# fskovbo/OptimalControlMPS

Hardware: NVIDIA B200
Metric: cost+gradient evals/s (BH N=20 chi=100) (higher is better)
Workload: dtype complex128 (f64)

## Files before the change

optimalcontrolmps_b200/csrc/decomp.cu:

```cuda
#include <cstdio>
#include <cstdlib>
#include "ocmps_internal.h"

__device__ unsigned long long g_jac_dbg[8];
__device__ double g_jac_flops[2];

namespace {

constexpr int JAC_THREADS = 512;
constexpr int JAC_EPL = 8;
constexpr int JAC_NV_SMEM = 512;
constexpr int JAC_MAX_SWEEPS = 60;
constexpr int JAC_BLOCKED_ROWS = 64;
constexpr double JAC_TOL2 = 1e-28;
constexpr double DEFLATE_REL = 1e-30;
constexpr int NV_MAX = 2048;
constexpr int BJ_C = 8;
constexpr int BJ_TPP = 4;
constexpr int BJ_MAX_ROWS = 256;
constexpr int BJ_SLOTS = BJ_MAX_ROWS / 2;
constexpr int BJ_THREADS = BJ_SLOTS * BJ_TPP;
constexpr int BJ_MAX_EPL = 8;
constexpr int BJ_MIN_CAP = 112;

// ... 1344 lines not shown
        if (act && redo) { tnew = tail; if (hl == 0) sh.nref[hv] = tail; }
      }
      if (act && hl == 0) sh.ncur[hv] = tnew > 0.0 ? tnew : 0.0;
    }
    __syncthreads();
    QB_MARK(3)
  }
#ifdef OCMPS_JAC_TRACE
  if (tid == 0 && rank == 0 && nv >= 24)
    printf("JTQ kind %d blk %d nv %d len %d keff %d qr %lld : exchange %lld pull %lld norm+scalars %lld update %lld\n", a.kind, blk, nv, len, keff,
           (long long)(clock64() - t_qr0), tp[0], tp[1], tp[2], tp[3]);
#endif
  const int ldz = nv;
  for (int vl = warp; vl < nown; vl += BJ_THREADS / 32) {
    const int i = sh.posof[v0 + vl];
    const cplx* y = Yv + (size_t)vl * len;
    for (int c = lane; c < keff; c += 32) {
      cplx v = make_double2(0.0, 0.0);
      if (c < i) v = y[c];
      else if (c == i) v = make_double2(sh.rdr[c], sh.rdi[c]);
      Yb[(size_t)c * ldz + i] = v;
    }
  }
  if (rank == 0) {
    short* gperm = reinterpret_cast<short*>(b.scratch_d + 4 * NV_MAX) + B.p_off;
    for (int i = tid; i < nv; i += BJ_THREADS) gperm[i] = sh.pos2phys[i];
    if (tid == 0) {
      double* hF = b.scratch_d + 7 * NV_MAX;
      int* hK = reinterpret_cast<int*>(b.scratch_d + 7 * NV_MAX + OCMPS_MAX_BLK);
      hF[blk] = F;
      hK[blk] = -1;
      if (nv >= 64) { const long long t_now = clock64(); atomicAdd(&g_jac_dbg[5], (unsigned long long)(t_now - t_qr0)); atomicAdd(&g_jac_dbg[7], (unsigned long long)(t_now - t_qr0)); }
      hK[OCMPS_MAX_BLK + blk] = keff;
      hK[2 * OCMPS_MAX_BLK + blk] = ldz;
      const double nn = (double)len, mmv = (double)nv;
      atomicAdd(&g_jac_flops[0], 8.0 * nn * nn * mmv + (56.0 / 3.0) * nn * nn * nn);
      if (blk == 0) {
        const double dn = mode == 0 ? (double)w->n : (double)w->m, dm = mode == 0 ? (double)w->m : (double)w->n;
        atomicAdd(&g_jac_flops[1], 8.0 * dn * dn * dm + (56.0 / 3.0) * dn * dn * dn);
      }
    }
  }
  clus::cluster_sync();
}

struct BjShared {
  double2 xbuf[2][BJ_C][BJ_SLOTS];
  unsigned long long mbar[2];
  double nrm[BJ_MAX_ROWS];
  int rot, big;
};

__device__ __forceinline__ double2 bj_exchange(BjShared& sh, unsigned& xcount, unsigned rank, int nslots, int slot, int lane, double x, double y) {
  const unsigned b = xcount & 1u, par = (xcount >> 1) & 1u;
  ++xcount;
  const unsigned mb = clus::smem_u32(&sh.mbar[b]);
  if (lane == 0 && slot < nslots) {
    sh.xbuf[b][rank][slot] = make_double2(x, y);
    const unsigned la = clus::smem_u32(&sh.xbuf[b][rank][slot]);
#pragma unroll
    for (unsigned p = 1; p < (unsigned)BJ_C; ++p) {
      const unsigned peer = (rank + p) % BJ_C;
      clus::st_async_v2(clus::mapa(la, peer), x, y, clus::mapa(mb, peer));
    }
  }
  clus::mbar_wait(mb, par);
  if (threadIdx.x == 0) clus::mbar_expect(mb, (unsigned)((BJ_C - 1) * nslots * 16));
  __syncwarp();
  double sx = 0.0, sy = 0.0;
  if (slot < nslots) {
#pragma unroll
    for (int r = 0; r < BJ_C; ++r) { const double2 v = sh.xbuf[b][r][slot]; sx += v.x; sy += v.y; }
  }
  return make_double2(sx, sy);
}

template <int TPP, int EPL>
__device__ void bj_run(DecompBuffers& b, const DecompBlock& B, int keff, int ldz, double F, cplx* __restrict__ Rs, BjShared& sh) {
  const int tid = threadIdx.x, slot = tid / TPP, lane = tid % TPP;
  const unsigned rank = clus::cluster_rank();
  const int nv = B.nv;
  const int w = (nv + BJ_C - 1) / BJ_C;
  const int c0 = (int)rank * w;
  constexpr int WP = (TPP * EPL) % 8 == 0 ? TPP * EPL + 4 : ((TPP * EPL) % 8 == 4 ? TPP * EPL : TPP * EPL + (12 - (TPP * EPL) % 8) % 8);
  const cplx* Yb = b.ywork + b.ywork_half + B.ws_off;
  cplx* Ya = b.ywork + B.ws_off;
  const short* perm = reinterpret_cast<const short*>(b.scratch_d + 4 * NV_MAX) + B.p_off;
  const double thr = F * DEFLATE_REL;
  unsigned xcount = 0;
  for (int e = tid; e < keff * WP; e += BJ_THREADS) {
    const int r = e / WP, cl = e % WP, c = c0 + cl;
    Rs[e] = (cl < w && c < nv) ? Yb[(size_t)r * ldz + c] : make_double2(0.0, 0.0);
  }
  __syncthreads();
  const int npad = (keff + 1) & ~1, nslots = npad >> 1, mm = npad - 1;
  cplx ra[EPL], rb[EPL];
  auto load_row = [&](cplx (&r)[EPL], int row) {
    const cplx* z = Rs + (row >= 0 ? row : 0) * WP + lane;
#pragma unroll
    for (int e = 0; e < EPL; ++e) r[e] = row >= 0 ? z[TPP * e] : make_double2(0.0, 0.0);
  };
  auto store_row = [&](const cplx (&r)[EPL], int row) {
    if (row < 0) return;
    cplx* z = Rs + row * WP + lane;
#pragma unroll
    for (int e = 0; e < EPL; ++e) z[TPP * e] = r[e];
  };
  auto lanes_sum = [&](double v) {
#pragma unroll
    for (int o = TPP / 2; o > 0; o >>= 1) v += __shfl_xor_sync(0xffffffffu, v, o);
    return v;
  };
  auto exact_norms = [&]() {
    const int x = 2 * slot < keff ? 2 * slot : -1, y = 2 * slot + 1 < keff ? 2 * slot + 1 : -1;
    load_row(ra, x);
    load_row(rb, y);
    double sa = 0.0, sb = 0.0;
#pragma unroll
    for (int e = 0; e < EPL; ++e) { sa += ra[e].x * ra[e].x + ra[e].y * ra[e].y; sb += rb[e].x * rb[e].x + rb[e].y * rb[e].y; }
    sa = lanes_sum(sa); sb = lanes_sum(sb);
    const double2 t = bj_exchange(sh, xcount, rank, nslots, slot, lane, sa, sb);
    if (lane == 0) { if (x >= 0) sh.nrm[x] = t.x; if (y >= 0) sh.nrm[y] = t.y; }
  };
  bool converged = keff < 2;
#ifdef OCMPS_JAC_TRACE
  long long tq[3] = {0, 0, 0};
  long long tql = clock64();
  int nrounds = 0;
#define BJ_MARK(i) { const long long tn = clock64(); tq[i] += tn - tql; tql = tn; }
#else
#define BJ_MARK(i)
#endif
  for (int sweep = 0; sweep < JAC_MAX_SWEEPS && !converged; ++sweep) {
    exact_norms();
    if (tid == 0) { sh.rot = 0; sh.big = 0; }
    __syncthreads();
    for (int R = 0; R < npad - 1; ++R) {
      int p = -1, q = -1;
      if (slot < nslots) {
        p = R + slot; if (p >= mm) p -= mm;
        q = R - slot; if (q < 0) q += mm;
        if (slot == 0) q = npad - 1;
        if (p > q) { const int t = p; p = q; q = t; }
        if (q >= keff) { p = -1; q = -1; }
      }
      const bool act = p >= 0;
      load_row(ra, p);
      load_row(rb, q);
      const double aa = act ? sh.nrm[p] : 0.0, bb = act ? sh.nrm[q] : 0.0;
      double c0r = 0.0, c0i = 0.0, c1r = 0.0, c1i = 0.0;
#pragma unroll
      for (int e = 0; e < EPL; ++e) {
        const double pr = ra[e].x * rb[e].x + ra[e].y * rb[e].y;
        const double pi = ra[e].x * rb[e].y - ra[e].y * rb[e].x;
        if (e & 1) { c1r += pr; c1i += pi; } else { c0r += pr; c0i += pi; }
      }
      const double pre = lanes_sum(c0r + c1r), pim = lanes_sum(c0i + c1i);
      BJ_MARK(0)
      const double2 cc = bj_exchange(sh, xcount, rank, nslots, slot, lane, pre, pim);
      BJ_MARK(1)
      if (act) {
        const double cre = cc.x, cim = cc.y;
        const double c2 = cre * cre + cim * cim;
        if (aa <= thr || bb <= thr) {
          if (aa <= thr && aa > 0.0) {
#pragma unroll
            for (int e = 0; e < EPL; ++e) ra[e] = make_double2(0.0, 0.0);
            store_row(ra, p);
            if (lane == 0) sh.nrm[p] = 0.0;
          }
          if (bb <= thr && bb > 0.0) {
#pragma unroll
            for (int e = 0; e < EPL; ++e) rb[e] = make_double2(0.0, 0.0);
            store_row(rb, q);
            if (lane == 0) sh.nrm[q] = 0.0;
          }
        } else if (c2 > JAC_TOL2 * aa * bb) {
          const double dd = 0.5 * (bb - aa);
          const double xh = dd * dd + c2;
          const double ih = rsqrt(xh);
          const double h = xh * ih;
          const double sdh = fabs(dd) + h;
          const double wv = rsqrt(2.0 * h * sdh);
          const double cs = sdh * wv;
          const double sgw = dd >= 0.0 ? wv : -wv;
          const double sr = sgw * cre, si = sgw * cim;
#pragma unroll
          for (int e = 0; e < EPL; ++e) {
            const cplx u = ra[e], v = rb[e];
            ra[e] = make_double2(cs * u.x - (sr * v.x + si * v.y), cs * u.y - (sr * v.y - si * v.x));
            rb[e] = make_double2(cs * v.x + (sr * u.x - si * u.y), cs * v.y + (sr * u.y + si * u.x));
          }
          store_row(ra, p);
          store_row(rb, q);
          if (lane == 0) {
            const double trr = c2 * (sgw * wv) * (2.0 * h);
            const double a1 = aa - trr, b1 = bb + trr;
            sh.nrm[p] = a1 > 0.0 ? a1 : 0.0;
            sh.nrm[q] = b1 > 0.0 ? b1 : 0.0;
            sh.rot = 1;
            if (c2 > 1e-16 * aa * bb) sh.big = 1;
          }
        }
      }
      __syncthreads();
      BJ_MARK(2)
#ifdef OCMPS_JAC_TRACE
      ++nrounds;
#endif
    }
    converged = (sh.rot == 0) || (sh.big == 0);
    __syncthreads();
    if (!converged && sweep == JAC_MAX_SWEEPS - 1 && tid == 0 && rank == 0) atomicOr(b.status, OCMPS_ST_NOCONV);
    if (tid == 0 && rank == 0) { atomicAdd(&g_jac_dbg[0], 1ull); atomicMax(&g_jac_dbg[2], (unsigned long long)(sweep + 1)); if (nv >= 64) atomicAdd(&g_jac_dbg[3], 1ull); if (nv >= 64 && sweep == 0) atomicAdd(&g_jac_dbg[4], 1ull); }
  }
#ifdef OCMPS_JAC_TRACE
  if (tid == 0 && rank == 0 && nv >= 24 && nrounds > 0)
    printf("JTB nv %d keff %d EPL %d rounds %d per round: load+dot %lld exchange %lld rotate+sync %lld\n", nv, keff, EPL, nrounds, tq[0] / nrounds, tq[1] / nrounds,
           tq[2] / nrounds);
#endif
  exact_norms();
  __syncthreads();
  for (int v = slot; v < nv; v += BJ_THREADS / TPP) {
    if (v < keff) {
      const double sq = sh.nrm[v];
      const double inv = sq > 0.0 ? rsqrt(sq) : 0.0;
      for (int cl = lane; cl < w; cl += TPP) {
        const int c = c0 + cl;
        if (c < nv) { const cplx u = Rs[v * WP + cl]; Ya[(size_t)v * nv + (int)perm[c]] = make_double2(u.x * inv, u.y * inv); }
      }
      if (lane == 0 && rank == 0) b.P[B.p_off + v] = sq;
    } else if (lane == 0 && rank == 0) {
      b.P[B.p_off + v] = 0.0;
    }
  }
}

__global__ void __launch_bounds__(BJ_THREADS) jacobi_big_kernel(DecompArgs a, DecompBuffers b) {
  extern __shared__ __align__(16) unsigned char smem_raw[];
  __shared__ BjShared sh;
  const DecompWork* w = b.dw;
  const int blk = blockIdx.x / BJ_C;
  if (blk >= w->nblocks) return;
  if (w->blk[blk].nv > BJ_MAX_ROWS || w->blk[blk].len > BJ_MAX_ROWS) return;
  const int* hK = reinterpret_cast<const int*>(b.scratch_d + 7 * NV_MAX + OCMPS_MAX_BLK);
  const int keff = hK[OCMPS_MAX_BLK + blk];
  if (keff < 0) return;
  const int ldz = hK[2 * OCMPS_MAX_BLK + blk];
  const DecompBlock B = w->blk[blk];
  const double F = (b.scratch_d + 7 * NV_MAX)[blk];
  const int tid = threadIdx.x;
  const int nslots = ((keff + 1) & ~1) >> 1;
  if (tid == 0) {
    clus::mbar_init(clus::smem_u32(&sh.mbar[0]), 1);
    clus::mbar_init(clus::smem_u32(&sh.mbar[1]), 1);
    asm volatile("fence.mbarrier_init.release.cluster;" ::: "memory");
    clus::mbar_expect(clus::smem_u32(&sh.mbar[0]), (unsigned)((BJ_C - 1) * nslots * 16));
    clus::mbar_expect(clus::smem_u32(&sh.mbar[1]), (unsigned)((BJ_C - 1) * nslots * 16));
  }
  __syncthreads();
  clus::cluster_sync();
  const long long t0 = clock64();
  cplx* Rs = reinterpret_cast<cplx*>(smem_raw);
  const int wcols = (B.nv + BJ_C - 1) / BJ_C;
  if (keff <= BJ_THREADS / 8 * 2) {
    switch ((wcols + 7) / 8) {
      case 1: bj_run<8, 1>(b, B, keff, ldz, F, Rs, sh); break;
      case 2: bj_run<8, 2>(b, B, keff, ldz, F, Rs, sh); break;
      case 3: bj_run<8, 3>(b, B, keff, ldz, F, Rs, sh); break;
      default: bj_run<8, 4>(b, B, keff, ldz, F, Rs, sh); break;
    }
  } else {
    switch ((wcols + 3) / 4) {
      case 1: bj_run<4, 1>(b, B, keff, ldz, F, Rs, sh); break;
      case 2: bj_run<4, 2>(b, B, keff, ldz, F, Rs, sh); break;
      case 3: bj_run<4, 3>(b, B, keff, ldz, F, Rs, sh); break;
      case 4: bj_run<4, 4>(b, B, keff, ldz, F, Rs, sh); break;
      case 5: bj_run<4, 5>(b, B, keff, ldz, F, Rs, sh); break;
      case 6: bj_run<4, 6>(b, B, keff, ldz, F, Rs, sh); break;
      case 7: bj_run<4, 7>(b, B, keff, ldz, F, Rs, sh); break;
      default: bj_run<4, 8>(b, B, keff, ldz, F, Rs, sh); break;
    }
  }
  clus::cluster_sync();
  if (tid == 0 && clus::cluster_rank() == 0) {
    atomicAdd(&g_jac_dbg[1], 1ull);
    const long long t1 = clock64();
    if (B.nv >= 64) { atomicAdd(&g_jac_dbg[6], (unsigned long long)(t1 - t0)); atomicAdd(&g_jac_dbg[7], (unsigned long long)(t1 - t0)); }
#ifdef OCMPS_JAC_TRACE
    if (B.nv >= 24) printf("JT3 kind %d blk %d nv %d keff %d jac %lld\n", a.kind, blk, B.nv, keff, (long long)(t1 - t0));
#endif
  }
}

constexpr int RC_C = 4;
constexpr int RC_NBLK = 2 * RC_C;
constexpr int RC_ROWS = JAC_BLOCKED_ROWS / RC_NBLK;
constexpr int RC_WORK_THREADS = 16 * RC_ROWS;
constexpr int RC_MIN_ROWS = 40;

__device__ unsigned long long g_rc_dbg[2];

struct RcShared {
  double nrm[2][2][RC_ROWS];
  int flags[2][RC_C];
  int rot, big;
};

__device__ __forceinline__ void rc_blocks(int R, int s, int& P, int& Q) {
  constexpr int mm = RC_NBLK - 1;
  int p = R + s; if (p >= mm) p -= mm;
  int q = R - s; if (q < 0) q += mm;
  if (s == 0) q = RC_NBLK - 1;
  P = p; Q = q;
}

__device__ __forceinline__ void rc_bar() { asm volatile("bar.sync 1, %0;" ::"n"(RC_WORK_THREADS) : "memory"); }

template <int EPL>
__device__ __forceinline__ void rc_block_round(cplx* __restrict__ Z0, cplx* __restrict__ Z1, double* n0, double* n1, int rb, int base0, int base1,
                                               int keff, double thr, bool intra, int* s_rot, int* s_big) {
  constexpr int ldz = 16 * EPL;
  const int tid = threadIdx.x, hl = tid & 15, h = tid >> 4;
  cplx ra[EPL], rb_[EPL];
  double na = 0.0, nb = 0.0;
  auto load_row = [&](cplx (&r)[EPL], double& n, const cplx* Z, const double* nz, int row) {
    const cplx* z = Z + (row >= 0 ? row : 0) * ldz + hl;
#pragma unroll
    for (int e = 0; e < EPL; ++e) r[e] = row >= 0 ? z[16 * e] : make_double2(0.0, 0.0);
    n = row >= 0 ? nz[row] : 0.0;
  };
  auto store_row = [&](const cplx (&r)[EPL], double n, cplx* Z, double* nz, int row) {
    cplx* z = Z + row * ldz + hl;
#pragma unroll
    for (int e = 0; e < EPL; ++e) z[16 * e] = r[e];
    if (hl == 0) nz[row] = n;
  };
  if (intra) {
    const int X = h / (RC_ROWS / 2), j = h % (RC_ROWS / 2);
    cplx* Z = X ? Z1 : Z0;
    double* nz = X ? n1 : n0;
    const int base = X ? base1 : base0;
    const int rbp = (rb + 1) & ~1, m = rbp - 1;
    for (int r = 0; r < m; ++r) {
      int p = r + j; if (p >= m) p -= m;
      int q = r - j; if (q < 0) q += m;
      if (j == 0) q = m;
      const bool act = 2 * j < rbp && p < rb && q < rb && base + p < keff && base + q < keff;
      load_row(ra, na, Z, nz, act ? p : -1);
      load_row(rb_, nb, Z, nz, act ? q : -1);
      jac_rotate<EPL>(ra, rb_, na, nb, act, thr, hl, s_rot, s_big);
      if (act) { store_row(ra, na, Z, nz, p); store_row(rb_, nb, Z, nz, q); }
      rc_bar();
    }
  }
  const bool has_a = h < rb && base0 + h < keff;
  load_row(ra, na, Z0, n0, has_a ? h : -1);
  for (int t = 0; t < rb; ++t) {
    int jb = h + t; if (jb >= rb) jb -= rb;
    const bool act = has_a && base1 + jb < keff;
    load_row(rb_, nb, Z1, n1, act ? jb : -1);
    jac_rotate<EPL>(ra, rb_, na, nb, act, thr, hl, s_rot, s_big);
    if (act) store_row(rb_, nb, Z1, n1, jb);
    rc_bar();
  }
  if (has_a) store_row(ra, na, Z0, n0, h);
}

template <int EPL>
__device__ __forceinline__ void rc_run(const DecompArgs& a, const DecompBuffers& b, int blk, int keff, unsigned rank, cplx* __restrict__ Zs, RcShared& sh) {
  constexpr int ldz = 16 * EPL;
  constexpr int BLK = RC_ROWS * ldz;
  const int tid = threadIdx.x, lane = tid & 31, warp = tid >> 5, nwarps = JAC_THREADS / 32;
  const DecompBlock B = b.dw->blk[blk];
  const int nv = B.nv;
  const int rb = (keff + RC_NBLK - 1) / RC_NBLK;
  const double F = (b.scratch_d + 7 * NV_MAX)[blk];
  const double thr = F * DEFLATE_REL;
  const cplx* Yb = b.ywork + b.ywork_half + B.ws_off;
  auto zb = [&](int buf, int k) { return Zs + (2 * buf + k) * BLK; };
  const long long t_jac0 = clock64();
  int P, Q;
  rc_blocks(0, (int)rank, P, Q);
  for (int e = tid; e < 2 * BLK; e += JAC_THREADS) {
    const int k = e / BLK, r = (e % BLK) / ldz, c = e % ldz;
    const int row = (k ? Q : P) * rb + r;
    Zs[e] = (r < rb && row < keff) ? Yb[row * ldz + c] : make_double2(0.0, 0.0);
  }
  __syncthreads();
  int cur = 0;
  bool done = false;
#ifdef OCMPS_JAC_TRACE
  long long t_work = 0, t_xchg = 0;
  int nrounds = 0, nxchg = 0;
#endif
  for (int sweep = 0; sweep < JAC_MAX_SWEEPS && !done; ++sweep) {
    for (int lr = warp; lr < 2 * RC_ROWS; lr += nwarps) {
      const int k = lr / RC_ROWS, r = lr % RC_ROWS;
      const cplx* y = zb(cur, k) + r * ldz;
      double s = 0.0;
      for (int c = lane; c < nv; c += 32) { const cplx u = y[c]; s += u.x * u.x + u.y * u.y; }
      s = warp_sum(s);
      if (lane == 0) sh.nrm[cur][k][r] = s;
    }
    if (tid == 0) { sh.rot = 0; sh.big = 0; }
    __syncthreads();
    for (int R = 0; R < RC_NBLK - 1; ++R) {
#ifdef OCMPS_JAC_TRACE
      const long long tw0 = clock64();
#endif
      if (tid < RC_WORK_THREADS) rc_block_round<EPL>(zb(cur, 0), zb(cur, 1), sh.nrm[cur][0], sh.nrm[cur][1], rb, P * rb, Q * rb, keff, thr, R == 0, &sh.rot, &sh.big);
      __syncthreads();
#ifdef OCMPS_JAC_TRACE
      const long long tw1 = clock64();
      t_work += tw1 - tw0;
      nrounds += rb + (R == 0 ? ((rb + 1) & ~1) - 1 : 0);
#endif
      const bool last = R == RC_NBLK - 2;
      if (last && tid < RC_C) {
        const int f = (sh.rot ? 1 : 0) | (sh.big ? 2 : 0);
        asm volatile("st.shared::cluster.u32 [%0], %1;" ::"r"(clus::mapa(clus::smem_u32(&sh.flags[sweep & 1][rank]), (unsigned)tid)), "r"(f) : "memory");
      }
      clus::cluster_sync();
      if (last) {
        int any = 0;
#pragma unroll
        for (int r = 0; r < RC_C; ++r) any |= sh.flags[sweep & 1][r];
        done = !(any & 1) || !(any & 2);
        if (tid == 0 && rank == 0) {
          atomicAdd(&g_jac_dbg[0], 1ull); atomicMax(&g_jac_dbg[2], (unsigned long long)(sweep + 1)); atomicAdd(&g_rc_dbg[1], 1ull);
          if (nv >= 64) atomicAdd(&g_jac_dbg[3], 1ull);
          if (nv >= 64 && sweep == 0) atomicAdd(&g_jac_dbg[4], 1ull);
          if (!done && sweep == JAC_MAX_SWEEPS - 1) atomicOr(b.status, OCMPS_ST_NOCONV);
        }
        if (done || sweep == JAC_MAX_SWEEPS - 1) break;
      }
      int NP, NQ;
      rc_blocks(last ? 0 : R + 1, (int)rank, NP, NQ);
      unsigned src0 = 0, src1 = 0, nsrc0 = 0, nsrc1 = 0;
      for (int s = 0; s < RC_C; ++s) {
        int p, q;
        rc_blocks(R, s, p, q);
        const unsigned zp = clus::mapa(clus::smem_u32(zb(cur, 0)), (unsigned)s), zq = clus::mapa(clus::smem_u32(zb(cur, 1)), (unsigned)s);
        const unsigned np = clus::mapa(clus::smem_u32(sh.nrm[cur][0]), (unsigned)s), nq = clus::mapa(clus::smem_u32(sh.nrm[cur][1]), (unsigned)s);
        if (p == NP) { src0 = zp; nsrc0 = np; }
        if (q == NP) { src0 = zq; nsrc0 = nq; }
        if (p == NQ) { src1 = zp; nsrc1 = np; }
        if (q == NQ) { src1 = zq; nsrc1 = nq; }
      }
      for (int e = tid; e < 2 * rb * ldz; e += JAC_THREADS) {
        const int k = e >= rb * ldz, o = e - k * rb * ldz;
        double xr, xi;
        asm volatile("ld.shared::cluster.v2.f64 {%0, %1}, [%2];" : "=d"(xr), "=d"(xi) : "r"((k ? src1 : src0) + (unsigned)o * 16u) : "memory");
        zb(cur ^ 1, k)[o] = make_double2(xr, xi);
      }
      if (tid < 2 * RC_ROWS) {
        const int k = tid / RC_ROWS, r = tid % RC_ROWS;
        double x;
        asm volatile("ld.shared::cluster.f64 %0, [%1];" : "=d"(x) : "r"((k ? nsrc1 : nsrc0) + (unsigned)r * 8u) : "memory");
        sh.nrm[cur ^ 1][k][r] = x;
      }
      __syncthreads();
#ifdef OCMPS_JAC_TRACE
      t_xchg += clock64() - tw1;
      ++nxchg;
#endif
      cur ^= 1; P = NP; Q = NQ;
    }
  }
  const long long t_jac1 = clock64();
  const short* perm = reinterpret_cast<const short*>(b.scratch_d + 4 * NV_MAX) + B.p_off;
  cplx* Ya = b.ywork + B.ws_off;
  for (int lr = warp; lr < 2 * RC_ROWS; lr += nwarps) {
    const int k = lr / RC_ROWS, r = lr % RC_ROWS, v = (k ? Q : P) * rb + r;
    if (r >= rb || v >= keff) continue;
    const cplx* y = zb(cur, k) + r * ldz;
    double s = 0.0;
    for (int c = lane; c < nv; c += 32) { const cplx u = y[c]; s += u.x * u.x + u.y * u.y; }
    s = warp_sum(s);
    const double inv = s > 0.0 ? rsqrt(s) : 0.0;
    for (int c = lane; c < nv; c += 32) {
      const cplx u = y[c];
      Ya[v * nv + (int)perm[c]] = make_double2(u.x * inv, u.y * inv);
    }
    if (lane == 0) b.P[B.p_off + v] = s;
  }
  if (rank == 0) for (int v = keff + tid; v < nv; v += JAC_THREADS) b.P[B.p_off + v] = 0.0;
  if (tid == 0 && rank == 0) {
    atomicAdd(&g_jac_dbg[1], 1ull);
    atomicAdd(&g_rc_dbg[0], 1ull);
    if (nv >= 64) {
      atomicAdd(&g_jac_dbg[6], (unsigned long long)(t_jac1 - t_jac0));
      atomicAdd(&g_jac_dbg[7], (unsigned long long)(t_jac1 - t_jac0));
    }
#ifdef OCMPS_JAC_TRACE
    if (nv >= 24)
      printf("JTR kind %d blk %d nv %d keff %d rb %d jac %lld : rotation rounds %d, %lld clk per round; block exchanges %d, %lld clk each\n", a.kind, blk, nv,
             keff, rb, t_jac1 - t_jac0, nrounds, nrounds ? t_work / nrounds : 0ll, nxchg, nxchg ? t_xchg / nxchg : 0ll);
#endif
  }
}

__global__ void __launch_bounds__(JAC_THREADS) jacobi_rows_cluster_kernel(DecompArgs a, DecompBuffers b, int smem_elems) {
  extern __shared__ __align__(16) unsigned char smem_raw[];
  __shared__ RcShared sh;
  const int blk = (int)blockIdx.x / RC_C;
  const unsigned rank = clus::cluster_rank();
  const int keff = rot_handover_rows(b, blk, smem_elems);
  if (keff < 0) return;
  if (keff < RC_MIN_ROWS) {
    if (rank == 0) jacobi_rot_block(a, b, blk, keff, smem_raw);
    return;
  }
  cplx* Zs = reinterpret_cast<cplx*>(smem_raw);
  switch ((b.dw->blk[blk].nv + 15) >> 4) {
    case 1: rc_run<1>(a, b, blk, keff, rank, Zs, sh); break;
    case 2: rc_run<2>(a, b, blk, keff, rank, Zs, sh); break;
    case 3: rc_run<3>(a, b, blk, keff, rank, Zs, sh); break;
    case 4: rc_run<4>(a, b, blk, keff, rank, Zs, sh); break;
    case 5: rc_run<5>(a, b, blk, keff, rank, Zs, sh); break;
    case 6: rc_run<6>(a, b, blk, keff, rank, Zs, sh); break;
    case 7: rc_run<7>(a, b, blk, keff, rank, Zs, sh); break;
    default: rc_run<8>(a, b, blk, keff, rank, Zs, sh); break;
  }
}

__global__ void __launch_bounds__(1024) truncate_kernel(DecompArgs a, DecompBuffers b, TruncParams tp) {
  __shared__ double cP[NV_MAX];
  __shared__ double sSorted[NV_MAX];
  __shared__ short cQ[NV_MAX], cI[NV_MAX], cI2[NV_MAX];
  __shared__ unsigned char sKeep[NV_MAX];
  __shared__ int sBlkOff[OCMPS_MAX_BLK + 1];
  __shared__ double sWarp[32];
  __shared__ int sWarpCnt[33];
  __shared__ double s_docut, s_kept;
  __shared__ int s_nfinal;
  DecompWork* w = b.dw;
  const int nv = w->nvtot;
  const int nblocks = w->nblocks;
  const int tid = threadIdx.x, lane = tid & 31, warp = tid >> 5;
  for (int i = tid; i < nblocks; i += blockDim.x) sBlkOff[i] = w->blk[i].p_off;
  if (tid == 0) { s_nfinal = 0; s_docut = 0.0; }
  const int i0 = 2 * tid, i1 = i0 + 1;
  const double p0 = i0 < nv ? b.P[i0] : 0.0, p1 = i1 < nv ? b.P[i1] : 0.0;
  const int f0 = p0 > 0.0, f1 = p1 > 0.0;
  int incl = f0 + f1;
#pragma unroll
  for (int o = 1; o < 32; o <<= 1) { const int up = __shfl_up_sync(0xffffffffu, incl, o); if (lane >= o) incl += up; }
  if (lane == 31) sWarpCnt[warp + 1] = incl;
  if (tid == 0) sWarpCnt[0] = 0;
  __syncthreads();
  if (warp == 0) {
    int v = sWarpCnt[lane + 1];
#pragma unroll
    for (int o = 1; o < 32; o <<= 1) { const int up = __shfl_up_sync(0xffffffffu, v, o); if (lane >= o) v += up; }
    sWarpCnt[lane + 1] = v;
  }
  __syncthreads();
  const int nnz = sWarpCnt[32];
  {
    int k = sWarpCnt[warp] + incl - f0 - f1;
    if (f0) { cP[k] = p0; cQ[k] = (short)b.vecq[i0]; cI[k] = (short)i0; ++k; }
    if (f1) { cP[k] = p1; cQ[k] = (short)b.vecq[i1]; cI[k] = (short)i1; }
  }
  __syncthreads();
  {
    int tpe = 1;
    while (tpe < 8 && nnz * tpe * 2 <= (int)blockDim.x) tpe *= 2;
    const int sub = tid & (tpe - 1);
    for (int k0 = 0; k0 < nnz; k0 += (int)blockDim.x / tpe) {
      const int k = k0 + tid / tpe;
      const bool in = k < nnz;
      const double pk = in ? cP[k] : 0.0;
      int rank = 0;
      if (in)
        for (int j = sub; j < nnz; j += tpe) {
          const double pj = cP[j];
          rank += (pj > pk) || (pj == pk && j < k);
        }
      for (int o = 1; o < tpe; o <<= 1) rank += __shfl_xor_sync(0xffffffffu, rank, o);
      if (in && sub == 0) sSorted[rank] = pk;
    }
  }
  __syncthreads();
  const int origm = nv;
  const int e0 = nnz - 1 - 2 * tid, e1 = e0 - 1;
  const double v0 = e0 >= 0 ? sSorted[e0] : 0.0, v1 = e1 >= 0 ? sSorted[e1] : 0.0;
  {
    double run = v0 + v1;
#pragma unroll
    for (int o = 1; o < 32; o <<= 1) { const double up = __shfl_up_sync(0xffffffffu, run, o); if (lane >= o) run += up; }
    if (lane == 31) sWarp[warp] = run;
    __syncthreads();
    if (warp == 0) {
      double ws = sWarp[lane];
#pragma unroll
      for (int o = 1; o < 32; o <<= 1) { const double up = __shfl_up_sync(0xffffffffu, ws, o); if (lane >= o) ws += up; }
      sWarp[lane] = ws;
    }
    __syncthreads();
    const double base = warp > 0 ? sWarp[warp - 1] : 0.0;
    const double inc = base + run;
    if (e0 >= 0) sSorted[e0] = inc - v1;
    if (e1 >= 0) sSorted[e1] = inc;
  }
  __syncthreads();
  {
    const double total_w = nnz > 0 ? sSorted[0] : 0.0;
    const double scale = tp.rel_cutoff ? (total_w == 0.0 ? 1.0 : total_w) : 1.0;
    const double cut = tp.cutoff * scale;
    const int nmax = (tp.maxm < origm ? tp.maxm : origm) - 1;
    int best = 0;
    if (cut <= 0.0) {
      best = nmax > 0 ? nmax : 0;
    } else {
      const int lim = nmax < nnz - 1 ? nmax : nnz - 1;
      for (int n = tid; n <= lim; n += blockDim.x)
        if (n < tp.minm || sSorted[n] >= cut) best = n > best ? n : best;
      if (tp.minm - 1 > best && tp.minm - 1 <= nmax) best = tp.minm - 1;
    }
    if (best > 0) atomicMax(&s_nfinal, best);
  }
  __syncthreads();
  {
    const int m = s_nfinal + 1;
    if (tid == 0) { sWarp[0] = 0.0; sWarp[1] = 0.0; }
    __syncthreads();
    if (e0 == m) sWarp[0] = v0;
    if (e1 == m) sWarp[0] = v1;
    if (e0 == m - 1) sWarp[1] = v0;
    if (e1 == m - 1) sWarp[1] = v1;
    __syncthreads();
    if (tid == 0) {
      double docut = 0.0;
      if (origm == 1) {
        docut = sWarp[1] / 2.0;
      } else if (origm > 1 && m < origm) {
        const double pm = sWarp[0], pm1 = sWarp[1];
        docut = (pm + pm1) / 2.0;
        if (fabs(pm - pm1) < 1e-3 * pm1) docut += 1e-3 * pm1;
      }
      s_docut = docut;
    }
    __syncthreads();
  }
  const double docut = s_docut;
  {
    const int ka = 2 * tid, kb = ka + 1;
    const int fa = ka < nnz && cP[ka] > docut, fb = kb < nnz && cP[kb] > docut;
    if (ka < nnz) sKeep[ka] = (unsigned char)fa;
    if (kb < nnz) sKeep[kb] = (unsigned char)fb;
    int inc = fa + fb;
#pragma unroll
    for (int o = 1; o < 32; o <<= 1) { const int up = __shfl_up_sync(0xffffffffu, inc, o); if (lane >= o) inc += up; }
    __syncthreads();
    if (lane == 31) sWarpCnt[warp + 1] = inc;
    if (tid == 0) sWarpCnt[0] = 0;
    __syncthreads();
    if (warp == 0) {
      int v = sWarpCnt[lane + 1];
#pragma unroll
      for (int o = 1; o < 32; o <<= 1) { const int up = __shfl_up_sync(0xffffffffu, v, o); if (lane >= o) v += up; }
      sWarpCnt[lane + 1] = v;
    }
    __syncthreads();
    const int base = sWarpCnt[warp] + inc - fa - fb;
    if (ka < nnz) cI2[ka] = (short)base;
    if (kb < nnz) cI2[kb] = (short)(base + fa);
  }
  __syncthreads();
  const int total = sWarpCnt[32];
  int* inv_blk = b.pos + NV_MAX;
  int* inv_v = b.pos + 2 * NV_MAX;
  double part = 0.0;
  for (int k = tid; k < nnz; k += blockDim.x) {
    if (!sKeep[k]) continue;
    const int qk = cQ[k];
    const double pk = cP[k];
    int rank = 0, j = k - 1;
    for (; j >= 0 && cQ[j] == qk; --j) rank += sKeep[j] && cP[j] >= pk;
    const int pos0 = cI2[j + 1];
    for (j = k + 1; j < nnz && cQ[j] == qk; ++j) rank += sKeep[j] && cP[j] > pk;
    const int pos = pos0 + rank;
    if (pos < tp.cap) {
      const int i = cI[k];
      a.qNew[pos] = qk;
      int bi = 0;
      while (bi + 1 < nblocks && sBlkOff[bi + 1] <= i) ++bi;
      inv_blk[pos] = bi;
      inv_v[pos] = i - sBlkOff[bi];
      part += pk;
    }
  }
  {
#pragma unroll
    for (int o = 16; o > 0; o >>= 1) part += __shfl_xor_sync(0xffffffffu, part, o);
    __syncthreads();
    if (lane == 0) sWarp[warp] = part;
    __syncthreads();
    if (tid == 0) {
      double t = 0.0;
      for (int i = 0; i < 32; ++i) t += sWarp[i];
      s_kept = t;
    }
    __syncthreads();
  }
  if (tid == 0) {
    int k = total;
    if (k == 0 && nv > 0) {
      k = 1;
      a.qNew[0] = b.vecq[0];
      inv_blk[0] = 0;
      inv_v[0] = 0;
    }
    if (k > tp.cap) { atomicOr(b.status, OCMPS_ST_CAPACITY); k = tp.cap; }
    w->newdim = k;
    *a.dimNew = k;
    const double kept = s_kept;
    double scale = 1.0;
    if (tp.normalize) {
      const double nrm = sqrt(kept);
      if (nrm > 1e-16) scale = 1.0 / nrm;
    }
    w->scale = scale;
    const int n = w->n, m = w->m;
    GemmDesc g1;
    g1.pad = 0;
    g1.A = g1.B = nullptr; g1.C = nullptr; g1.M = g1.N = g1.K = 0; g1.lda = g1.ldb = g1.ldc = 1; g1.opA = g1.opB = 0;
    if (a.kind == DK_ORTH_LEFT) {
      const int far = a.D * (*a.dimNb);
      g1.A = a.partner; g1.opA = 0; g1.lda = m;
      g1.B = a.nb_in; g1.opB = 0; g1.ldb = far;
      g1.C = a.nb_out; g1.ldc = far; g1.M = k; g1.N = far; g1.K = m;
    } else if (a.kind == DK_ORTH_RIGHT) {
      const int far = a.D * (*a.dimNb);
      g1.A = a.nb_in; g1.opA = 0; g1.lda = n;
      g1.B = a.partner; g1.opB = 0; g1.ldb = k;
      g1.C = a.nb_out; g1.ldc = k; g1.M = far; g1.N = k; g1.K = n;
    }
    b.descs[1] = g1;
  }
}

constexpr int BUILD_THREADS = 512;
__global__ void __launch_bounds__(BUILD_THREADS) build_factors_kernel(DecompArgs a, DecompBuffers b) {
  extern __shared__ __align__(16) unsigned char bsm[];
  __shared__ double red[BUILD_THREADS / 32];
  __shared__ double s_inv;
  const DecompWork* w = b.dw;
  const int k = w->newdim;
  const int kk = blockIdx.x;
  if (kk >= k) return;
  const int n = w->n, m = w->m, ld = w->ld, mode = w->mode;
  const int* comp_blk = b.comp_idx + NV_MAX;
  const int* comp_rank = b.comp_idx + 2 * NV_MAX;
  const int* vec_blk = b.vec_idx + NV_MAX;
  const int* vec_rank = b.vec_idx + 2 * NV_MAX;
  const int bi = b.pos[NV_MAX + kk], j = b.pos[2 * NV_MAX + kk];
  const DecompBlock B = w->blk[bi];
  const int nv = B.nv, len = B.len;
  const cplx* Zj = b.ywork + B.ws_off + (size_t)j * nv;
  const double sigma = sqrt(b.P[B.p_off + j]) * w->scale;
  cplx* zs = reinterpret_cast<cplx*>(bsm);
  cplx* out = zs + nv;
  int* vidx = reinterpret_cast<int*>(out + len);
  int* cidx = vidx + nv;
  const int tid = threadIdx.x, lane = tid & 31, wp = tid >> 5;
  constexpr int NW = BUILD_THREADS / 32;
  for (int v = tid; v < nv; v += BUILD_THREADS) { zs[v] = Zj[v]; vidx[v] = b.vec_idx[B.vec_off + v]; }
  for (int c = tid; c < len; c += BUILD_THREADS) cidx[c] = b.comp_idx[B.comp_off + c];
// ... 328 lines not shown
```

Baseline: 0.9277.

## Replace per-round cluster barrier with push-based st.async exchange and mbarrier handshakes

Measured after the change: 0.9425, median of 6. 1.6% higher.

```diff
diff --git a/optimalcontrolmps_b200/csrc/decomp.cu b/optimalcontrolmps_b200/csrc/decomp.cu
--- a/optimalcontrolmps_b200/csrc/decomp.cu
+++ b/optimalcontrolmps_b200/csrc/decomp.cu
@@ -1670,7 +1670,9 @@
 __device__ unsigned long long g_rc_dbg[2];
 
 struct RcShared {
+  unsigned long long full[2];
   double nrm[2][2][RC_ROWS];
+  unsigned freed[RC_C];
   int flags[2][RC_C];
   int rot, big;
 };
@@ -1681,6 +1683,27 @@
   int q = R - s; if (q < 0) q += mm;
   if (s == 0) q = RC_NBLK - 1;
   P = p; Q = q;
+}
+
+__device__ __forceinline__ void rc_holder(int R, int X, int& s, int& k) {
+  s = 0; k = 0;
+  for (int r = 0; r < RC_C; ++r) {
+    int p, q;
+    rc_blocks(R, r, p, q);
+    if (p == X) { s = r; k = 0; }
+    if (q == X) { s = r; k = 1; }
+  }
+}
+
+template <int EPL>
+__device__ __forceinline__ unsigned rc_in_bytes(int Rn, int rank, int rb) {
+  const int Rp = Rn == 0 ? RC_NBLK - 2 : Rn - 1;
+  int P, Q, s, k;
+  rc_blocks(Rn, rank, P, Q);
+  unsigned n = 0;
+  rc_holder(Rp, P, s, k); if (s != rank) ++n;
+  rc_holder(Rp, Q, s, k); if (s != rank) ++n;
+  return n * (unsigned)(rb * 16 * EPL * 16 + RC_ROWS * 8);
 }
 
 __device__ __forceinline__ void rc_bar() { asm volatile("bar.sync 1, %0;" ::"n"(RC_WORK_THREADS) : "memory"); }
@@ -1748,6 +1771,14 @@
   const cplx* Yb = b.ywork + b.ywork_half + B.ws_off;
   auto zb = [&](int buf, int k) { return Zs + (2 * buf + k) * BLK; };
   const long long t_jac0 = clock64();
+  if (tid == 0) {
+    clus::mbar_init(clus::smem_u32(&sh.full[0]), 1);
+    clus::mbar_init(clus::smem_u32(&sh.full[1]), 1);
+    asm volatile("fence.mbarrier_init.release.cluster;" ::: "memory");
+    clus::mbar_expect(clus::smem_u32(&sh.full[1]), rc_in_bytes<EPL>(1, (int)rank, rb));
+    clus::mbar_expect(clus::smem_u32(&sh.full[0]), rc_in_bytes<EPL>(2 % (RC_NBLK - 1), (int)rank, rb));
+  }
+  if (tid < RC_C) sh.freed[tid] = 1u;
   int P, Q;
   rc_blocks(0, (int)rank, P, Q);
   for (int e = tid; e < 2 * BLK; e += JAC_THREADS) {
@@ -1756,7 +1787,9 @@
     Zs[e] = (r < rb && row < keff) ? Yb[row * ldz + c] : make_double2(0.0, 0.0);
   }
   __syncthreads();
+  asm volatile("barrier.cluster.arrive.release.aligned;" ::: "memory");
   int cur = 0;
+  unsigned xg = 0;
   bool done = false;
 #ifdef OCMPS_JAC_TRACE
   long long t_work = 0, t_xchg = 0;
@@ -1777,20 +1810,33 @@
 #ifdef OCMPS_JAC_TRACE
       const long long tw0 = clock64();
 #endif
-      if (tid < RC_WORK_THREADS) rc_block_round<EPL>(zb(cur, 0), zb(cur, 1), sh.nrm[cur][0], sh.nrm[cur][1], rb, P * rb, Q * rb, keff, thr, R == 0, &sh.rot, &sh.big);
+      const bool last = R == RC_NBLK - 2;
+      const int Rn = last ? 0 : R + 1;
+      int d0, k0, d1, k1;
+      rc_holder(Rn, P, d0, k0);
+      rc_holder(Rn, Q, d1, k1);
+      if (tid < RC_WORK_THREADS) {
+        rc_block_round<EPL>(zb(cur, 0), zb(cur, 1), sh.nrm[cur][0], sh.nrm[cur][1], rb, P * rb, Q * rb, keff, thr, R == 0, &sh.rot, &sh.big);
+      } else if (tid == RC_WORK_THREADS && (d0 != (int)rank || d1 != (int)rank)) {
+        const unsigned fa0 = clus::smem_u32(&sh.freed[d0]), fa1 = clus::smem_u32(&sh.freed[d1]);
+        unsigned f0, f1;
+        do {
+          asm volatile("ld.acquire.cluster.shared::cta.u32 %0, [%1];" : "=r"(f0) : "r"(fa0) : "memory");
+          asm volatile("ld.acquire.cluster.shared::cta.u32 %0, [%1];" : "=r"(f1) : "r"(fa1) : "memory");
+        } while ((d0 != (int)rank && f0 <= xg) || (d1 != (int)rank && f1 <= xg));
+      }
       __syncthreads();
 #ifdef OCMPS_JAC_TRACE
       const long long tw1 = clock64();
       t_work += tw1 - tw0;
       nrounds += rb + (R == 0 ? ((rb + 1) & ~1) - 1 : 0);
 #endif
-      const bool last = R == RC_NBLK - 2;
-      if (last && tid < RC_C) {
-        const int f = (sh.rot ? 1 : 0) | (sh.big ? 2 : 0);
-        asm volatile("st.shared::cluster.u32 [%0], %1;" ::"r"(clus::mapa(clus::smem_u32(&sh.flags[sweep & 1][rank]), (unsigned)tid)), "r"(f) : "memory");
-      }
-      clus::cluster_sync();
       if (last) {
+        if (tid < RC_C) {
+          const int f = (sh.rot ? 1 : 0) | (sh.big ? 2 : 0);
+          asm volatile("st.shared::cluster.u32 [%0], %1;" ::"r"(clus::mapa(clus::smem_u32(&sh.flags[sweep & 1][rank]), (unsigned)tid)), "r"(f) : "memory");
+        }
+        clus::cluster_sync();
         int any = 0;
 #pragma unroll
         for (int r = 0; r < RC_C; ++r) any |= sh.flags[sweep & 1][r];
@@ -1802,38 +1848,59 @@
           if (!done && sweep == JAC_MAX_SWEEPS - 1) atomicOr(b.status, OCMPS_ST_NOCONV);
         }
         if (done || sweep == JAC_MAX_SWEEPS - 1) break;
-      }
-      int NP, NQ;
-      rc_blocks(last ? 0 : R + 1, (int)rank, NP, NQ);
-      unsigned src0 = 0, src1 = 0, nsrc0 = 0, nsrc1 = 0;
-      for (int s = 0; s < RC_C; ++s) {
-        int p, q;
-        rc_blocks(R, s, p, q);
-        const unsigned zp = clus::mapa(clus::smem_u32(zb(cur, 0)), (unsigned)s), zq = clus::mapa(clus::smem_u32(zb(cur, 1)), (unsigned)s);
-        const unsigned np = clus::mapa(clus::smem_u32(sh.nrm[cur][0]), (unsigned)s), nq = clus::mapa(clus::smem_u32(sh.nrm[cur][1]), (unsigned)s);
-        if (p == NP) { src0 = zp; nsrc0 = np; }
-        if (q == NP) { src0 = zq; nsrc0 = nq; }
-        if (p == NQ) { src1 = zp; nsrc1 = np; }
-        if (q == NQ) { src1 = zq; nsrc1 = nq; }
-      }
-      for (int e = tid; e < 2 * rb * ldz; e += JAC_THREADS) {
-        const int k = e >= rb * ldz, o = e - k * rb * ldz;
-        double xr, xi;
-        asm volatile("ld.shared::cluster.v2.f64 {%0, %1}, [%2];" : "=d"(xr), "=d"(xi) : "r"((k ? src1 : src0) + (unsigned)o * 16u) : "memory");
-        zb(cur ^ 1, k)[o] = make_double2(xr, xi);
-      }
-      if (tid < 2 * RC_ROWS) {
-        const int k = tid / RC_ROWS, r = tid % RC_ROWS;
-        double x;
-        asm volatile("ld.shared::cluster.f64 %0, [%1];" : "=d"(x) : "r"((k ? nsrc1 : nsrc0) + (unsigned)r * 8u) : "memory");
-        sh.nrm[cur ^ 1][k][r] = x;
+      } else if (xg == 0) {
+        asm volatile("barrier.cluster.wait.acquire.aligned;" ::: "memory");
+      }
+      const unsigned z0 = clus::mapa(clus::smem_u32(zb(cur ^ 1, k0)), (unsigned)d0), z1 = clus::mapa(clus::smem_u32(zb(cur ^ 1, k1)), (unsigned)d1);
+      const unsigned m0 = clus::mapa(clus::smem_u32(&sh.full[cur ^ 1]), (unsigned)d0), m1 = clus::mapa(clus::smem_u32(&sh.full[cur ^ 1]), (unsigned)d1);
+      {
+        constexpr int NPT = (2 * BLK + JAC_THREADS - 1) / JAC_THREADS;
+        const int nel = rb * ldz;
+        cplx v[NPT];
+#pragma unroll
+        for (int i = 0; i < NPT; ++i) {
+          const int e = tid + i * JAC_THREADS, k = e >= nel, o = e - k * nel;
+          if (e < 2 * nel) v[i] = zb(cur, k)[o];
+        }
+#pragma unroll
+        for (int i = 0; i < NPT; ++i) {
+          const int e = tid + i * JAC_THREADS, k = e >= nel, o = e - k * nel;
+          if (e >= 2 * nel) break;
+          const int d = k ? d1 : d0;
+          if (d == (int)rank) zb(cur ^ 1, k ? k1 : k0)[o] = v[i];
+          else clus::st_async_v2((k ? z1 : z0) + (unsigned)o * 16u, v[i].x, v[i].y, k ? m1 : m0);
+        }
+        if (tid < 2 * RC_ROWS) {
+          const int k = tid / RC_ROWS, r = tid % RC_ROWS, d = k ? d1 : d0, kk = k ? k1 : k0;
+          const double x = sh.nrm[cur][k][r];
+          if (d == (int)rank) {
+            sh.nrm[cur ^ 1][kk][r] = x;
+          } else {
+            const unsigned na = clus::mapa(clus::smem_u32(&sh.nrm[cur ^ 1][kk][r]), (unsigned)d);
+            asm volatile("st.async.weak.shared::cluster.mbarrier::complete_tx::bytes.f64 [%0], %1, [%2];" ::"r"(na), "d"(x), "r"(k ? m1 : m0) : "memory");
+          }
+        }
       }
       __syncthreads();
+      if (tid < 2) {
+        const int Rnn = Rn == RC_NBLK - 2 ? 0 : Rn + 1;
+        int NNP, NNQ, s, k;
+        rc_blocks(Rnn, (int)rank, NNP, NNQ);
+        rc_holder(Rn, tid ? NNQ : NNP, s, k);
+        if (s != (int)rank)
+          asm volatile("st.release.cluster.shared::cluster.u32 [%0], %1;" ::"r"(clus::mapa(clus::smem_u32(&sh.freed[rank]), (unsigned)s)), "r"(xg + 2) : "memory");
+      }
+      clus::mbar_wait(clus::smem_u32(&sh.full[cur ^ 1]), (xg >> 1) & 1u);
+      if (tid == 0) {
+        const int Rnnn = (Rn + 2) % (RC_NBLK - 1);
+        clus::mbar_expect(clus::smem_u32(&sh.full[cur ^ 1]), rc_in_bytes<EPL>(Rnnn, (int)rank, rb));
+      }
 #ifdef OCMPS_JAC_TRACE
       t_xchg += clock64() - tw1;
       ++nxchg;
 #endif
-      cur ^= 1; P = NP; Q = NQ;
+      rc_blocks(Rn, (int)rank, P, Q);
+      cur ^= 1; ++xg;
     }
   }
   const long long t_jac1 = clock64();
```
